# hjsuh94/irs_mpc

Hardware: AMD Instinct MI355X
Metric: rollouts*timesteps/s (randomized-smoothing pass) + iLQR-iters/s (higher is better)
Workload: dtype f32

## Files before the change

### irs_mpc_amd/csrc/ctrlbox_mfma.hip

```cpp
#include "boxqp.hpp"

namespace {

typedef double v4d __attribute__((ext_vector_type(4)));
typedef const __attribute__((address_space(1))) double* gptr_d;

constexpr int kPdasIterM = 10;
constexpr int kPdasSingleM = 50;
#ifndef IRS_LAZY_MIN
#define IRS_LAZY_MIN 6
#endif
constexpr int kLazyPrefixMin = IRS_LAZY_MIN;
constexpr int KIND_ABS_M = 0, KIND_REL_M = 1;

__device__ __forceinline__ double fast_rcp_m(double d) {
    double r = __builtin_amdgcn_rcp(d);
    r = fma(fma(-d, r, 1.0), r, r);
    r = fma(fma(-d, r, 1.0), r, r);
    return r;
}
__device__ __forceinline__ double readlane_d(double v, int src) {
    const int lo = __builtin_amdgcn_readlane(__double2loint(v), src);
    const int hi = __builtin_amdgcn_readlane(__double2hiint(v), src);
    return __hiloint2double(hi, lo);
}
template <int N>
__device__ __forceinline__ double row_newbcast_d(double v) {
    int lo = __double2loint(v), hi = __double2hiint(v);
    lo = __builtin_amdgcn_update_dpp(0, lo, 0x150 + N, 0xf, 0xf, true);
    hi = __builtin_amdgcn_update_dpp(0, hi, 0x150 + N, 0xf, 0xf, true);
    return __hiloint2double(hi, lo);
}
__device__ __forceinline__ double wmax_d(double v) {
#pragma unroll
    for (int s = 32; s >= 1; s >>= 1) v = fmax(v, __shfl_xor(v, s, 64));
    return v;
}
__device__ __forceinline__ double wmin_d(double v) {
#pragma unroll
    for (int s = 32; s >= 1; s >>= 1) v = fmin(v, __shfl_xor(v, s, 64));
    return v;
}
__device__ __forceinline__ int wmax_i(int v) {
#pragma unroll
    for (int s = 32; s >= 1; s >>= 1) v = max(v, __shfl_xor(v, s, 64));
    return v;
}
__device__ __forceinline__ int wmin_i(int v) {
#pragma unroll
    for (int s = 32; s >= 1; s >>= 1) v = min(v, __shfl_xor(v, s, 64));
    return v;
}

template <int NR, int M>
struct MfLayout {
    static constexpr int NS = NR + M, NH = NS + 1, NHP = (NH + 3) / 4 * 4, KA = NHP / 4;
    static constexpr bool FITS = NHP + M <= 16 && M <= 4;
    static constexpr int GR = NHP + M, GT = KA * 4 * GR, PT = KA * 4 * NHP;
    static __host__ __device__ size_t oG(int) { return 0; }
    static __host__ __device__ size_t oP(int T) { return (size_t)T * GT; }
    static __host__ __device__ size_t oV(int T) { return oP(T) + (size_t)(T + 1) * PT; }
    static __host__ __device__ size_t oQ(int T) { return oV(T) + (size_t)7 * T * M; }
    static __host__ __device__ size_t oS(int T) { return oQ(T) + (size_t)(T + 1) * NR; }
    static __host__ __device__ size_t rec_doubles(int T) { return oS(T) + (size_t)T; }
    static constexpr int small = 2 * NR * NR + M * M + NH + M + 16 + 128;
};

template <class Model, int KIND, bool LDSREC>
__global__ __launch_bounds__(128) void ctrlbox_mfma_kernel(BoxArgs a, double* gws, long long* stamps) {
    constexpr int NR = Model::NX, M = Model::NU;
    using L = MfLayout<NR, M>;
    constexpr int NS = L::NS, NH = L::NH, NHP = L::NHP, KA = L::KA, RN = L::KA;
    static_assert(L::FITS, "one 16 x 16 tile");
    constexpr double INF = __builtin_huge_val();
    extern __shared__ double lds[];
    const int T = a.T, lane = threadIdx.x & 63, col = lane & 15, rg = lane >> 4;
    const int wave = __builtin_amdgcn_readfirstlane((int)(threadIdx.x >> 6));
    const double tol_ = a.eps;
#ifdef IRS_CBM_STAMPS
    long long st_acc[24] = {0, 0, 0, 0, 0, 0, 0, 0, 0, 0, 0, 0, 0, 0, 0, 0, 0, 0, 0, 0, 0, 0, 0, 0};
#define CBM_MARK(k) do { const long long st_now = __builtin_amdgcn_s_memtime(); st_acc[k] += st_now - st_mark; st_mark = st_now; } while (0)
#define CBM_T0() const long long st_t0 = __builtin_amdgcn_s_memtime()
#define CBM_ADD(k, n) do { st_acc[k] += __builtin_amdgcn_s_memtime() - st_t0; st_acc[(k) + 1] += (n); } while (0)
#else
#define CBM_T0() do {} while (0)
#define CBM_MARK(k) do {} while (0)
#define CBM_ADD(k, n) do {} while (0)
#endif

    double* rec = LDSREC ? lds : gws;
    double* sm = LDSREC ? lds + L::rec_doubles(T) : lds;
    double* Gt = rec + L::oG(T);
    double* Pt = rec + L::oP(T);
    double* Vv = rec + L::oV(T);
    double* act_ = Vv;
    double* lo_ = Vv + (size_t)T * M;
    double* hi_ = Vv + (size_t)2 * T * M;
    double* uu_ = Vv + (size_t)3 * T * M;
    double* us_ = Vv + (size_t)4 * T * M;
    double* mu_ = Vv + (size_t)5 * T * M;
    double* bnd_ = Vv + (size_t)6 * T * M;
    double* qsd = rec + L::oQ(T);
    double* sig_ = rec + L::oS(T);
    double* Qsym = sm;
    double* Qdsym = Qsym + NR * NR;
    double* Rsym = Qdsym + NR * NR;
    double* sstart = Rsym + M * M;
    double* uctl = sstart + NH;
    double* junk = uctl + M + 16;

    auto rsync = [&]() {
        if constexpr (LDSREC) {
            asm volatile("s_waitcnt lgkmcnt(0)" ::: "memory");
        } else {
            __builtin_amdgcn_fence(__ATOMIC_RELEASE, "workgroup");
            asm volatile("s_waitcnt vmcnt(0) lgkmcnt(0)" ::: "memory");
            __builtin_amdgcn_fence(__ATOMIC_ACQUIRE, "workgroup");
        }
        __builtin_amdgcn_wave_barrier();
    };

    auto wg_barrier = [&]() {
        asm volatile("s_waitcnt vmcnt(0) lgkmcnt(0)" ::: "memory");
        __builtin_amdgcn_s_barrier();
        asm volatile("" ::: "memory");
    };

    if (wave == 1) {
        double xr[NR], ur[M], xn[NR], up[M], ub[M];
        if (lane == 0 && a.cost) *reinterpret_cast<unsigned long long*>(a.cost) = 0x7ff8000000000000ull;
#pragma unroll
        for (int i = 0; i < NR; ++i) xr[i] = a.x0[i];
#pragma unroll
        for (int j = 0; j < M; ++j) up[j] = 0.0;
        if (lane == 0) {
#pragma unroll
            for (int i = 0; i < NR; ++i) a.x_new[i] = xr[i];
        }
        auto quad = [&](const double* Wq, const double* e, int Kd) -> double {
            double q = 0.0;
            for (int i = 0; i < Kd; ++i)
                for (int j = 0; j < Kd; ++j) q += e[i] * Wq[i * Kd + j] * e[j];
            return q;
        };
        auto publish_start = [&]() {
#pragma unroll
            for (int j = 0; j < M; ++j) {
                double v = xr[0];
#pragma unroll
                for (int i = 1; i < NR; ++i) v = (i == Model::u_into_x(j)) ? xr[i] : v;
                ub[j] = v;
            }
            if (lane < NH) {
                double v = xr[0];
#pragma unroll
                for (int i = 1; i < NR; ++i) v = (i == lane) ? xr[i] : v;
#pragma unroll
                for (int j = 0; j < M; ++j) v = (NR + j == lane) ? ub[j] : v;
                sstart[lane] = lane == NS ? 1.0 : v;
            }
        };
        double cost = 0.0;
        unsigned warm = ~0u;
        irs_step_prepared<Model> pre;
        wg_barrier();
        publish_start();
        double xs[NR], dv[M];
        auto book = [&](int tau) {
            double e[NR];
#pragma unroll
            for (int i = 0; i < NR; ++i) e[i] = xs[i] - a.xd[(size_t)tau * NR + i];
            cost += quad(Qsym, e, NR) + quad(Rsym, dv, M);
            if (lane == 0) {
#pragma unroll
                for (int j = 0; j < M; ++j) a.u_new[(size_t)tau * M + j] = up[j];
#pragma unroll
                for (int i = 0; i < NR; ++i) a.x_new[(size_t)(tau + 1) * NR + i] = xr[i];
            }
        };
        for (int tau = 0; tau < T; ++tau) {
            wg_barrier();
            if (tau > 0) book(tau - 1);
            irs_step_along_prepare<Model>(a.p, xr, warm, pre);
            wg_barrier();
#pragma unroll
            for (int j = 0; j < M; ++j) ur[j] = KIND == KIND_ABS_M ? uctl[j] : ub[j] + uctl[j];
#pragma unroll
            for (int j = 0; j < M; ++j) dv[j] = ur[j] - (tau == 0 ? ub[j] : up[j]);
#pragma unroll
            for (int i = 0; i < NR; ++i) xs[i] = xr[i];
            irs_step_along_finish<Model>(a.p, xr, ur, pre, xn, &warm);
#pragma unroll
            for (int i = 0; i < NR; ++i) xr[i] = xn[i];
#pragma unroll
            for (int j = 0; j < M; ++j) up[j] = ur[j];
            publish_start();
        }
        book(T - 1);
        {
            double e[NR];
#pragma unroll
            for (int i = 0; i < NR; ++i) e[i] = xr[i] - a.xd[(size_t)T * NR + i];
            cost += quad(Qdsym, e, NR);
        }
        if (lane == 0 && a.cost) a.cost[0] = cost;
        return;
    }

    if (lane == 0) {
        a.info[0] = -1; a.info[1] = -1; a.info[2] = -1;
    }
    for (int q = lane; q < NR * NR; q += 64) {
        const int i = q / NR, j = q % NR;
        Qsym[q] = 0.5 * (a.Q[i * NR + j] + a.Q[j * NR + i]);
        Qdsym[q] = 0.5 * (a.Qd[i * NR + j] + a.Qd[j * NR + i]);
    }
    for (int q = lane; q < M * M; q += 64) {
        const int i = q / M, j = q % M;
        Rsym[q] = 0.5 * (a.R[i * M + j] + a.R[j * M + i]);
    }
    asm volatile("s_waitcnt lgkmcnt(0)" ::: "memory");
    __builtin_amdgcn_wave_barrier();
    const double* blo = KIND == KIND_ABS_M ? a.ulo : a.dlo;
    const double* bhi = KIND == KIND_ABS_M ? a.uhi : a.dhi;
    const int bs = KIND == KIND_ABS_M ? a.su : a.sd;
    for (int q = lane; q < T * M; q += 64) {
        const double lo = blo ? blo[(size_t)(q / M) * bs + q % M] : -INF;
        const double hi = bhi ? bhi[(size_t)(q / M) * bs + q % M] : INF;
        lo_[q] = lo;
        hi_[q] = hi;
        double a0 = a.act_io ? a.act_io[q] : 0.0;
        a0 = a0 < 0.0 ? (lo > -INF ? -1.0 : 0.0) : (a0 > 0.0 ? (hi < INF ? 1.0 : 0.0) : 0.0);
        act_[q] = a0;
        bnd_[q] = a0 < 0.0 ? lo : hi;
        uu_[q] = 0.0; us_[q] = 0.0; mu_[q] = 0.0;
    }
    for (int q = lane; q < (T + 1) * NR; q += 64) {
        const int t = q / NR, i = q % NR;
        double s = 0.0;
        for (int j = 0; j < NR; ++j) s += Qsym[i * NR + j] * a.xd[(size_t)t * NR + j];
        qsd[q] = -s;
    }
    for (size_t q = lane; q < (size_t)T * L::GT; q += 64) Gt[q] = 0.0;
    for (int q = lane; q < T; q += 64) sig_[q] = -1.0;
    auto Ru = [&](int i, int j) { return Rsym[i * M + j]; };
    v4d Lc;
#pragma unroll
    for (int r = 0; r < 4; ++r) {
        const int row = rg + 4 * r;
        double v = 0.0;
        if (row < NR && col < NR) v = Qsym[row * NR + col];
        else if (row >= NHP && row < NHP + M && col >= NHP && col < NHP + M) v = Ru(row - NHP, col - NHP);
        if (KIND == KIND_ABS_M) {
            if (row >= NR && row < NS && col >= NR && col < NS) v = Ru(row - NR, col - NR);
            else if (row >= NR && row < NS && col >= NHP && col < NHP + M) v = -Ru(row - NR, col - NHP);
            else if (col >= NR && col < NS && row >= NHP && row < NHP + M) v = -Ru(row - NHP, col - NR);
        }
        Lc[r] = v;
    }
    if (col < NHP) {
#pragma unroll
        for (int r = 0; r < KA; ++r) {
            const int row = rg + 4 * r;
            double v = 0.0;
            if (row < NR && col < NR) v = Qdsym[row * NR + col];
            else if ((col == NS && row < NR) || (row == NS && col < NR)) {
                const int i = col == NS ? row : col;
                for (int j = 0; j < NR; ++j) v -= Qdsym[i * NR + j] * a.xd[(size_t)T * NR + j];
            }
            Pt[(size_t)T * L::PT + (r * 4 + rg) * NHP + col] = v;
        }
    }
    rsync();

    gptr_d fp[5];
    int fstr[5];
    double fc[5];
    bool fld[5];
    {
        const gptr_d gA = (gptr_d)a.At, gB = (gptr_d)a.Bt, gc_ = (gptr_d)a.ct;
#pragma unroll
        for (int r = 0; r < 5; ++r) { fp[r] = gc_; fstr[r] = 0; fc[r] = 0.0; fld[r] = false; }
#pragma unroll
        for (int r = 0; r < 4; ++r) {
            const int row = rg + 4 * r;
            if (row < NR) {
                if (col < NR) { fp[r] = gA + row * NR + col; fstr[r] = NR * NR; fld[r] = true; }
                else if (col < NS) {
                    if (KIND == KIND_REL_M) { fp[r] = gB + row * M + (col - NR); fstr[r] = NR * M; fld[r] = true; }
                } else if (col == NS) { fp[r] = gc_ + row; fstr[r] = NR; fld[r] = true; }
                else if (col >= NHP && col < NHP + M) { fp[r] = gB + row * M + (col - NHP); fstr[r] = NR * M; fld[r] = true; }
            } else if (row < NS) {
                if (KIND == KIND_REL_M && col == row) fc[r] = 1.0;
                else if (col == NHP + (row - NR)) fc[r] = 1.0;
            } else if (row == NS && col == NS) {
                fc[r] = 1.0;
            }
        }
        if (rg < M) {
            if (col < NR) { fp[4] = gB + col * M + rg; fstr[4] = NR * M; fld[4] = true; }
            else if (col < NS) fc[4] = (col - NR) == rg ? 1.0 : 0.0;
        }
    }
    auto load_F = [&](int t, double* v) {
#pragma unroll
        for (int r = 0; r < 5; ++r) v[r] = fp[r][(long)t * fstr[r]];
    };
    auto finish_F = [&](const double* v, v4d& F, double& Ba) {
#pragma unroll
        for (int r = 0; r < 4; ++r) F[r] = fld[r] ? v[r] : fc[r];
        Ba = fld[4] ? v[4] : fc[4];
    };
    int qidx[KA];
    bool qhas[KA];
#pragma unroll
    for (int r = 0; r < KA; ++r) {
        const int row = rg + 4 * r;
        qhas[r] = (col == NS && row < NR) || (row == NS && col < NR);
        qidx[r] = qhas[r] ? (col == NS ? row : col) : 0;
    }

    int bad = 0;
    auto backward_sweep = [&](int t_hi, int t_lo) {
        if (t_hi < t_lo) return;
        CBM_T0();
        v4d P = {0.0, 0.0, 0.0, 0.0};
        if (col < NHP) {
#pragma unroll
            for (int r = 0; r < KA; ++r) P[r] = Pt[(size_t)(t_hi + 1) * L::PT + (r * 4 + rg) * NHP + col];
        }
        struct Pre { double Fraw[5]; double ac[M], bd[M], q[KA]; };
        auto load_step = [&](int t, Pre& p) {
            load_F(t, p.Fraw);
#pragma unroll
            for (int j = 0; j < M; ++j) {
                p.ac[j] = act_[(size_t)t * M + j];
                p.bd[j] = bnd_[(size_t)t * M + j];
            }
#pragma unroll
            for (int r = 0; r < KA; ++r) p.q[r] = qsd[(size_t)t * NR + qidx[r]];
        };
        bool pend = false;
        int pend_t = 0;
        v4d pendAcl = {0.0, 0.0, 0.0, 0.0};
        double pendGk = 0.0;
        auto flush_P = [&]() {
            double* pp = col < NHP ? Pt + (size_t)pend_t * L::PT + (size_t)rg * NHP + col : junk + lane;
            const int ps = col < NHP ? 4 * NHP : 0;
#pragma unroll
            for (int r = 0; r < KA; ++r) pp[r * ps] = P[r];
        };
        auto flush_G = [&]() {
            double* G = Gt + (size_t)pend_t * L::GT;
            double* gq = col < NH ? G + (size_t)col * L::GR + rg : junk + 64 + lane;
            const int gs = col < NH ? 4 : 0;
#pragma unroll
            for (int r = 0; r < KA; ++r) gq[r * gs] = pendAcl[r];
            double* gk = (col < NH && rg < M) ? G + (size_t)col * L::GR + NHP + rg : junk + 64 + lane;
            *gk = pendGk;
        };
        auto bw_step = [&](int t, const Pre& cur, Pre& nxt, bool prefetch) {
#ifdef IRS_CBM_STAMPS
            {
                const long long w0 = __builtin_amdgcn_s_memtime();
                asm volatile("s_waitcnt vmcnt(0)" ::: "memory");
                st_acc[7] += __builtin_amdgcn_s_memtime() - w0;
            }
#endif
#ifdef IRS_CBM_STAMPS
            long long st_mark = __builtin_amdgcn_s_memtime();
#endif
            v4d F;
            double Ba;
            finish_F(cur.Fraw, F, Ba);
            double ac[M], bb[M];
#pragma unroll
            for (int j = 0; j < M; ++j) {
                ac[j] = cur.ac[j];
                bb[j] = cur.bd[j];
            }
            v4d Lt = Lc;
            v4d D1 = {0.0, 0.0, 0.0, 0.0};
            v4d Th;
            if constexpr (LDSREC && KA == 3) {
                D1 = __builtin_amdgcn_mfma_f64_16x16x4f64(P[0], F[0], D1, 0, 0, 0);
                if (pend) flush_P();
                __builtin_amdgcn_sched_barrier(0);
                D1 = __builtin_amdgcn_mfma_f64_16x16x4f64(P[1], F[1], D1, 0, 0, 0);
                if (pend) flush_G();
                __builtin_amdgcn_sched_barrier(0);
                D1 = __builtin_amdgcn_mfma_f64_16x16x4f64(P[2], F[2], D1, 0, 0, 0);
                if (prefetch) load_F(t - 1, nxt.Fraw);
#pragma unroll
                for (int r = 0; r < KA; ++r) Lt[r] = qhas[r] ? cur.q[r] : Lc[r];
                __builtin_amdgcn_sched_barrier(0);
                Th = __builtin_amdgcn_mfma_f64_16x16x4f64(F[0], D1[0], Lt, 0, 0, 0);
                if (prefetch) {
#pragma unroll
                    for (int j = 0; j < M; ++j) {
                        nxt.ac[j] = act_[(size_t)(t - 1) * M + j];
                        nxt.bd[j] = bnd_[(size_t)(t - 1) * M + j];
                    }
                }
                __builtin_amdgcn_sched_barrier(0);
                Th = __builtin_amdgcn_mfma_f64_16x16x4f64(F[1], D1[1], Th, 0, 0, 0);
                if (prefetch) {
#pragma unroll
                    for (int r = 0; r < KA; ++r) nxt.q[r] = qsd[(size_t)(t - 1) * NR + qidx[r]];
                }
                __builtin_amdgcn_sched_barrier(0);
                Th = __builtin_amdgcn_mfma_f64_16x16x4f64(F[2], D1[2], Th, 0, 0, 0);
            } else if constexpr (LDSREC && KA == 2) {
                D1 = __builtin_amdgcn_mfma_f64_16x16x4f64(P[0], F[0], D1, 0, 0, 0);
                if (pend) flush_P();
                __builtin_amdgcn_sched_barrier(0);
                D1 = __builtin_amdgcn_mfma_f64_16x16x4f64(P[1], F[1], D1, 0, 0, 0);
                if (pend) flush_G();
                if (prefetch) load_F(t - 1, nxt.Fraw);
#pragma unroll
                for (int r = 0; r < KA; ++r) Lt[r] = qhas[r] ? cur.q[r] : Lc[r];
                __builtin_amdgcn_sched_barrier(0);
                Th = __builtin_amdgcn_mfma_f64_16x16x4f64(F[0], D1[0], Lt, 0, 0, 0);
                if (prefetch) {
#pragma unroll
                    for (int j = 0; j < M; ++j) {
                        nxt.ac[j] = act_[(size_t)(t - 1) * M + j];
                        nxt.bd[j] = bnd_[(size_t)(t - 1) * M + j];
                    }
#pragma unroll
                    for (int r = 0; r < KA; ++r) nxt.q[r] = qsd[(size_t)(t - 1) * NR + qidx[r]];
                }
                __builtin_amdgcn_sched_barrier(0);
                Th = __builtin_amdgcn_mfma_f64_16x16x4f64(F[1], D1[1], Th, 0, 0, 0);
            } else {
#pragma unroll
                for (int r = 0; r < KA; ++r) Lt[r] = qhas[r] ? cur.q[r] : Lc[r];
                if (prefetch) load_step(t - 1, nxt);
                if constexpr (LDSREC) {
                    D1 = __builtin_amdgcn_mfma_f64_16x16x4f64(P[0], F[0], D1, 0, 0, 0);
                    if (pend) flush_P();
                    __builtin_amdgcn_sched_barrier(0);
                    if constexpr (KA >= 2) D1 = __builtin_amdgcn_mfma_f64_16x16x4f64(P[1], F[1], D1, 0, 0, 0);
                    if (pend) flush_G();
                    __builtin_amdgcn_sched_barrier(0);
#pragma unroll
                    for (int s = 2; s < KA; ++s) D1 = __builtin_amdgcn_mfma_f64_16x16x4f64(P[s], F[s], D1, 0, 0, 0);
                } else {
#pragma unroll
                    for (int s = 0; s < KA; ++s) D1 = __builtin_amdgcn_mfma_f64_16x16x4f64(P[s], F[s], D1, 0, 0, 0);
                }
                Th = Lt;
#pragma unroll
                for (int s = 0; s < KA; ++s) Th = __builtin_amdgcn_mfma_f64_16x16x4f64(F[s], D1[s], Th, 0, 0, 0);
            }
            asm volatile("" :: "v"(Th[0]), "v"(Th[RN]));
            CBM_MARK(8);
            bool allpin = true;
#pragma unroll
            for (int j = 0; j < M; ++j) allpin = allpin && ac[j] != 0.0;
            double Kb = 0.0;
            bool my_free = false;
            if (__builtin_amdgcn_readfirstlane((int)allpin)) {
#pragma unroll
                for (int i = 0; i < M; ++i)
                    if (i == rg) Kb = col == NS ? bb[i] : 0.0;
                if constexpr (LDSREC) {
                    double* sp = lane == 0 ? sig_ + t : junk + lane;
                    *sp = 1.0;
                } else if (lane == 0) {
                    sig_[t] = 1.0;
                }
                CBM_MARK(9);
            } else {
                double H[M][M], gc[M], mf[M], bz[M];
                const v4d zero4 = {0.0, 0.0, 0.0, 0.0};
                const v4d Gc = __builtin_amdgcn_mfma_f64_16x16x4f64(rg == (col >> 2) ? 1.0 : 0.0, Th[RN], zero4, 0, 0, 0);
                auto bc = [&](double v, int j) {
                    switch (j) {
                        case 0: return row_newbcast_d<NHP + 0>(v);
                        case 1: return row_newbcast_d<(NHP + 1) & 15>(v);
                        case 2: return row_newbcast_d<(NHP + 2) & 15>(v);
                        default: return row_newbcast_d<(NHP + 3) & 15>(v);
                    }
                };
#pragma unroll
                for (int i = 0; i < M; ++i) {
#pragma unroll
                    for (int j = i; j < M; ++j) {
                        H[i][j] = bc(Gc[i], j);
                        H[j][i] = H[i][j];
                    }
                    gc[i] = Gc[i];
                    mf[i] = ac[i] == 0.0 ? 1.0 : 0.0;
                    bz[i] = ac[i] == 0.0 ? 0.0 : bb[i];
                }
                asm volatile("" :: "v"(H[0][0]), "v"(gc[0]), "v"(gc[M - 1]));
                CBM_MARK(9);
                double Hm[M][M], Hi[M][M], y[M];
    #pragma unroll
                for (int i = 0; i < M; ++i)
    #pragma unroll
                    for (int j = 0; j < M; ++j) Hm[i][j] = H[i][j];
                bool anypin = false;
    #pragma unroll
                for (int j = 0; j < M; ++j) anypin = anypin || ac[j] != 0.0;
                const bool pins = __builtin_amdgcn_readfirstlane((int)anypin) != 0;
                if (pins) {
    #pragma unroll
                    for (int i = 0; i < M; ++i)
    #pragma unroll
                        for (int j = 0; j < M; ++j) Hm[i][j] = i == j ? (ac[i] == 0.0 ? H[i][i] : 1.0) : H[i][j] * (mf[i] * mf[j]);
                }
                const double hsel = col == NS ? 1.0 : 0.0;
                double rhs[M];
    #pragma unroll
                for (int i = 0; i < M; ++i) {
                    rhs[i] = gc[i];
                }
                if (pins) {
    #pragma unroll
                    for (int i = 0; i < M; ++i) {
                        double hb0 = 0.0, hb1 = 0.0;
    #pragma unroll
                        for (int l = 0; l < M; ++l) {
                            if (l & 1) hb1 = fma(H[i][l], bz[l], hb1);
                            else hb0 = fma(H[i][l], bz[l], hb0);
                        }
                        rhs[i] = fma(hsel, hb0 + hb1, gc[i]) * mf[i];
                    }
                }
                bool spd = true;
                auto inv2 = [&](double p, double q, double r, double& ip, double& iq, double& ir) {
                    const double det = fma(p, r, -q * q);
                    spd = spd && p > 0.0 && det > 0.0;
                    const double id = fast_rcp_m(det);
                    ip = r * id; iq = -q * id; ir = p * id;
                };
                if constexpr (M == 1) {
                    spd = Hm[0][0] > 0.0;
                    Hi[0][0] = fast_rcp_m(Hm[0][0]);
                } else if constexpr (M == 2) {
                    inv2(Hm[0][0], Hm[0][1], Hm[1][1], Hi[0][0], Hi[0][1], Hi[1][1]);
                    Hi[1][0] = Hi[0][1];
                } else {
                    static_assert(M == 1 || M == 2 || M == 4, "closed-form inverse for 1, 2 or 4 controls");
                    double a0, a1, a2;
                    inv2(Hm[0][0], Hm[0][1], Hm[1][1], a0, a1, a2);
                    const double w00 = fma(a0, Hm[0][2], a1 * Hm[1][2]), w01 = fma(a0, Hm[0][3], a1 * Hm[1][3]);
                    const double w10 = fma(a1, Hm[0][2], a2 * Hm[1][2]), w11 = fma(a1, Hm[0][3], a2 * Hm[1][3]);
                    const double s00 = Hm[2][2] - fma(Hm[0][2], w00, Hm[1][2] * w10);
                    const double s01 = Hm[2][3] - fma(Hm[0][2], w01, Hm[1][2] * w11);
                    const double s11 = Hm[3][3] - fma(Hm[0][3], w01, Hm[1][3] * w11);
                    double c0, c1, c2;
                    inv2(s00, s01, s11, c0, c1, c2);
                    const double t0 = fma(a0, rhs[0], a1 * rhs[1]), t1 = fma(a1, rhs[0], a2 * rhs[1]);
                    const double q0 = rhs[2] - fma(Hm[0][2], t0, Hm[1][2] * t1);
                    const double q1 = rhs[3] - fma(Hm[0][3], t0, Hm[1][3] * t1);
                    y[2] = fma(c0, q0, c1 * q1);
                    y[3] = fma(c1, q0, c2 * q1);
                    y[0] = t0 - fma(w00, y[2], w01 * y[3]);
                    y[1] = t1 - fma(w10, y[2], w11 * y[3]);
                }
                if (!spd && bad == 0) bad = t + 1;
                if constexpr (M != 4) {
    #pragma unroll
                    for (int i = 0; i < M; ++i) {
                        double y0 = 0.0, y1 = 0.0;
    #pragma unroll
                        for (int l = 0; l < M; ++l) {
                            if (l & 1) y1 = fma(Hi[i][l], rhs[l], y1);
                            else y0 = fma(Hi[i][l], rhs[l], y0);
                        }
                        y[i] = y0 + y1;
                    }
                }
                double mfree = 0.0;
    #pragma unroll
                for (int i = 0; i < M; ++i) {
                    const double kv = hsel * bz[i] - y[i];
                    if (i == rg) { Kb = kv; mfree = mf[i]; }
                }
                if (rg >= M || col >= NH) Kb = 0.0;
                my_free = mfree != 0.0;
            }
            asm volatile("" :: "v"(Kb));
            CBM_MARK(10);
            v4d D = __builtin_amdgcn_mfma_f64_16x16x4f64(Th[RN], Kb, Th, 0, 0, 0);
            v4d Pn = __builtin_amdgcn_mfma_f64_16x16x4f64(Kb, D[RN], D, 0, 0, 0);
            v4d Acl = __builtin_amdgcn_mfma_f64_16x16x4f64(Ba, Kb, F, 0, 0, 0);
#pragma unroll
            for (int r = 0; r < 4; ++r) {
                const int row = rg + 4 * r;
                if constexpr (NH == NHP) P[r] = r < KA ? Pn[r] : 0.0;
                else P[r] = (r < KA && row < NH && col < NH) ? Pn[r] : 0.0;
            }
            double* G = Gt + (size_t)t * L::GT;
            if constexpr (LDSREC) {
                pend = true;
                pend_t = t;
                pendAcl = Acl;
                pendGk = my_free ? Kb : D[RN];
            } else {
                if (col < NHP) {
#pragma unroll
                    for (int r = 0; r < KA; ++r) Pt[(size_t)t * L::PT + (r * 4 + rg) * NHP + col] = P[r];
                }
                if (col < NH) {
#pragma unroll
                    for (int r = 0; r < KA; ++r) G[col * L::GR + (rg + 4 * r)] = Acl[r];
                    if (rg < M) G[col * L::GR + (NHP + rg)] = my_free ? Kb : D[RN];
                }
            }
            asm volatile("" :: "v"(P[0]));
            CBM_MARK(11);
        
        };
        Pre pa, pb;
        load_step(t_hi, pa);
        int t = t_hi;
        for (; t - 1 >= t_lo; t -= 2) {
            bw_step(t, pa, pb, true);
            bw_step(t - 1, pb, pa, t - 2 >= t_lo);
        }
        if (t >= t_lo) bw_step(t, pa, pb, false);
        if constexpr (LDSREC) {
            if (pend) {
                flush_P();
                flush_G();
            }
        }
        rsync();
        CBM_ADD(0, t_hi - t_lo + 1);
    };

    auto policy_rollout = [&](int t0, double* dst, int te, bool clip = false) {
        CBM_T0();
        v4d S = {0.0, 0.0, 0.0, 0.0};
        if (col == 0) {
#pragma unroll
            for (int s = 0; s < KA; ++s) {
                const int k = rg + 4 * s;
                S[s] = k < NH ? sstart[k] : 0.0;
            }
        }
        const int gofs = col < L::GR ? col : 0;
        const bool out_lane = col == 0 && rg < M;
        const int cj = rg < M ? rg : 0;
        struct Fw { double g[KA]; double ti, lo, hi, ac; };
        auto roll_range = [&](int ta, int tb, v4d& S, bool clipping) {
            const double* gp = Gt + (size_t)ta * L::GT + (size_t)rg * L::GR + gofs;
            int tq = ta;
            auto fetch = [&](Fw& f) {
#pragma unroll
                for (int s = 0; s < KA; ++s) f.g[s] = gp[4 * s * L::GR];
                gp += L::GT;
                if (clipping) {
                    f.ti = (double)tq;
                    f.lo = lo_[(size_t)tq * M + cj];
                    f.hi = hi_[(size_t)tq * M + cj];
                    f.ac = act_[(size_t)tq * M + cj];
                    ++tq;
                }
            };
            double* mo = (out_lane || !LDSREC) ? mu_ + (size_t)ta * M + (rg < M ? rg : 0) : junk + lane;
            const int mstride = (out_lane || !LDSREC) ? M : 0;
            auto emit = [&](const v4d& Dp) {
                if constexpr (LDSREC) *mo = Dp[RN];
                else if (out_lane) *mo = Dp[RN];
                mo += mstride;
            };
            auto step = [&](const Fw& f, const v4d& Sin, v4d& Sout, bool has_prev) {
                v4d Dn = {0.0, 0.0, 0.0, 0.0};
                Dn = __builtin_amdgcn_mfma_f64_16x16x4f64(col < L::GR ? f.g[0] : 0.0, Sin[0], Dn, 0, 0, 0);
                if (has_prev) emit(Sin);
#pragma unroll
                for (int s = 1; s < KA; ++s)
                    Dn = __builtin_amdgcn_mfma_f64_16x16x4f64(col < L::GR ? f.g[s] : 0.0, Sin[s], Dn, 0, 0, 0);
                if (clipping) {
                    const double raw = Dn[RN];
                    const double cl = fmin(fmax(raw, f.lo), f.hi);
                    const double dlt = (out_lane && f.ac == 0.0) ? cl - raw : 0.0;
                    if (__ballot(dlt != 0.0) != 0ull) {
                        const double bav = fp[4][(long)(int)f.ti * fstr[4]];
                        Dn = __builtin_amdgcn_mfma_f64_16x16x4f64(fld[4] ? bav : fc[4], dlt, Dn, 0, 0, 0);
                    }
                }
                Sout = Dn;
            };
            Fw fa, fb;
            v4d S1;
            fetch(fa);
            int t = ta;
            bool hp = false;
            for (; t + 1 < tb; t += 2) {
                fetch(fb);
                step(fa, S, S1, hp);
                if (t + 2 < tb) fetch(fa);
                step(fb, S1, S, true);
                hp = true;
            }
            if (t < tb) {
                step(fa, S, S1, hp);
                emit(S1);
                S = S1;
            } else if (hp) {
                emit(S);
            }
        };
#ifdef IRS_CBM_STAMPS
        const long long st_fl0 = __builtin_amdgcn_s_memtime();
#endif
        if (!clip) {
            roll_range(t0, te, S, false);
        } else {
            #ifndef IRS_KCHECK
#define IRS_KCHECK 16
#endif
            constexpr int kCheck = IRS_KCHECK;
            int t = t0;
            bool found = false;
            while (t < te && !found) {
                const int tc = min(t + kCheck, te);
                const v4d Ssave = S;
                roll_range(t, tc, S, false);
#ifdef IRS_CBM_STAMPS
                st_acc[20] += tc - t;
                st_acc[21] += 1;
#endif
                rsync();
                bool v = false;
                for (int q = t * M + lane; q < tc * M; q += 64) {
                    const double raw = mu_[q];
                    v = v || (act_[q] == 0.0 && (raw < lo_[q] || raw > hi_[q]));
                }
                if (__any(v)) {
                    S = Ssave;
                    found = true;
                } else {
                    t = tc;
                }
            }
#ifdef IRS_CBM_STAMPS
            st_acc[19] += te - t;
#endif
            if (t < te) roll_range(t, te, S, true);
        }
#ifdef IRS_CBM_STAMPS
        asm volatile("" :: "v"(S[0]));
        st_acc[13] += __builtin_amdgcn_s_memtime() - st_fl0;
        st_acc[12] += 1;
#endif
        rsync();
        for (int q = t0 * M + lane; q < te * M; q += 64) {
            const double raw = mu_[q], ac = act_[q];
            const double bd = bnd_[q];
            dst[q] = ac == 0.0 ? raw : bd;
            mu_[q] = ac == 0.0 ? 0.0 : raw;
        }
        rsync();
        CBM_ADD(2, te - t0);
    };

    auto saturated_start = [&](int t0) {
        v4d S = {0.0, 0.0, 0.0, 0.0};
        if (col == 0) {
#pragma unroll
            for (int s = 0; s < KA; ++s) {
                const int k = rg + 4 * s;
                S[s] = k < NH ? sstart[k] : 0.0;
            }
        }
        const gptr_d gB = (gptr_d)a.Bt;
        for (int t = t0; t < T; ++t) {
            const double* G = Gt + (size_t)t * L::GT;
            v4d Dn = {0.0, 0.0, 0.0, 0.0};
#pragma unroll
            for (int s = 0; s < KA; ++s) {
                const double g = col < L::GR ? G[(4 * s + rg) * L::GR + (col < L::GR ? col : 0)] : 0.0;
                Dn = __builtin_amdgcn_mfma_f64_16x16x4f64(g, S[s], Dn, 0, 0, 0);
            }
            double dlt[M];
#pragma unroll
            for (int j = 0; j < M; ++j) {
                const double v = readlane_d(Dn[RN], 16 * j);
                const double lo = lo_[(size_t)t * M + j], hi = hi_[(size_t)t * M + j];
                const double c = fmin(fmax(v, lo), hi);
                dlt[j] = c - v;
                if (lane == 0) {
                    act_[(size_t)t * M + j] = v < lo - tol_ ? -1.0 : (v > hi + tol_ ? 1.0 : 0.0);
                    bnd_[(size_t)t * M + j] = v < lo - tol_ ? lo : hi;
                    sig_[t] = -1.0;
                }
            }
            if (col == 0) {
#pragma unroll
                for (int s = 0; s < KA; ++s) {
                    const int row = rg + 4 * s;
                    double corr = 0.0;
                    if (row < NR) {
#pragma unroll
                        for (int j = 0; j < M; ++j) corr += gB[((size_t)t * NR + row) * M + j] * dlt[j];
                    } else if (row < NS) {
#pragma unroll
                        for (int j = 0; j < M; ++j) corr = (row - NR == j) ? dlt[j] : corr;
                    }
                    S[s] = Dn[s] + corr;
                }
            }
        }
        rsync();
    };

#ifdef IRS_CBM_STAMPS
    const long long st_begin = __builtin_amdgcn_s_memtime();
#endif
    int it_max = 0, n_fail = 0;
    const double tol = a.eps;
    bool full = true;
    wg_barrier();

    for (int tau = 0; tau < T; ++tau) {
        {
            CBM_T0();
            wg_barrier();
            CBM_ADD(4, 1);
        }
        const int t0 = tau;
        if (tau == 0) {
            bool any = false;
            for (int q = lane; q < T * M; q += 64) any = any || act_[q] != 0.0;
            if (!__any(any)) {
                backward_sweep(T - 1, 0);
                saturated_start(0);
            }
        }
        int t_dirty = full ? T - 1 : t0 - 1;
        int iters = 0;
        bool conv = false;
        int stale_hi = t0 - 1;
        auto prefix_end = [&]() {
            int pe = t0 - 1;
            for (int base = t0; base < T; base += 64) {
                const int t = base + lane;
                bool ok = false;
                if (t < T) {
                    bool allp = sig_[t] == 1.0;
#pragma unroll
                    for (int j = 0; j < M; ++j) allp = allp && act_[(size_t)t * M + j] != 0.0;
                    ok = allp;
                }
                const unsigned long long bal = __ballot(ok);
                const int run = bal == ~0ull ? 64 : __builtin_ctzll(~bal);
                pe = base + run - 1;
                if (run < 64) break;
            }
            return pe;
        };
        for (int it = 0; it < kPdasIterM + kPdasSingleM && !conv; ++it) {
            ++iters;
            const bool single = it >= kPdasIterM;
            int pe = t0 - 1;
            if (KIND == KIND_ABS_M && max(t_dirty, stale_hi) >= t0) {
                pe = prefix_end();
                if (pe - t0 + 1 < kLazyPrefixMin) pe = t0 - 1;
            }
            {
                const int hi = max(t_dirty, stale_hi), lo = max(t0, pe + 1);
                if (hi >= lo) backward_sweep(hi, lo);
                if (hi >= t0) stale_hi = lo - 1;
            }
            policy_rollout(t0, uu_, T, KIND == KIND_ABS_M);
            int chg = -1;
            double rworst = 0.0;
            int rq = 0x7fffffff;
            for (int qb = t0 * M; qb < T * M; qb += 64) {
                const int q = qb + lane;
                bool changed = false;
                if (q < T * M) {
                    const double ac = act_[q], u = uu_[q], mu = mu_[q];
                    const bool fresh = q / M > stale_hi;
                    double nw = ac;
                    if (ac == 0.0) {
                        if (u < lo_[q] - tol) nw = -1.0;
                        else if (u > hi_[q] + tol) nw = 1.0;
                    } else if (ac < 0.0) {
                        if (fresh && mu < -tol) nw = 0.0;
                    } else {
                        if (fresh && mu > tol) nw = 0.0;
                    }
                    if (single && nw == 0.0 && ac != 0.0) {
                        const double v = fabs(mu);
                        if (v > rworst) { rworst = v; rq = q; }
                        nw = ac;
                    }
                    changed = nw != ac;
                    if (changed) { act_[q] = nw; bnd_[q] = nw < 0.0 ? lo_[q] : hi_[q]; sig_[q / M] = -1.0; }
                }
                const unsigned long long cb = __ballot(changed);
                if (cb != 0ull) chg = max(chg, (qb + 63 - __builtin_clzll(cb)) / M);
            }
            if (single) {
                const double wm = wmax_d(rworst);
                if (wm > 0.0) {
                    const int qw = wmin_i(rworst == wm ? rq : 0x7fffffff);
                    if (lane == 0) { act_[qw] = 0.0; sig_[qw / M] = -1.0; }
                    chg = max(chg, qw / M);
                }
            }
            rsync();
            if (chg < 0 && stale_hi >= t0) {
                const int ph = stale_hi;
#ifdef IRS_CBM_STAMPS
                st_acc[14] += ph - t0 + 1;
#endif
                backward_sweep(ph, t0);
                stale_hi = t0 - 1;
                policy_rollout(t0, uu_, ph + 1);
                for (int qb = t0 * M; qb < (ph + 1) * M; qb += 64) {
                    const int q = qb + lane;
                    bool rel = false;
                    if (q < (ph + 1) * M) {
                        const double ac = act_[q], mu = mu_[q];
                        rel = (ac < 0.0 && mu < -tol) || (ac > 0.0 && mu > tol);
                        if (rel) { act_[q] = 0.0; sig_[q / M] = -1.0; }
                    }
                    const unsigned long long cb = __ballot(rel);
                    if (cb != 0ull) chg = max(chg, (qb + 63 - __builtin_clzll(cb)) / M);
                }
                rsync();
#ifdef IRS_CBM_STAMPS
                st_acc[15] += chg >= 0 ? 1 : 0;
#endif
            }
            if (chg < 0) conv = true;
            else t_dirty = chg;
        }
        if (stale_hi >= t0) { t_dirty = max(t_dirty, stale_hi); stale_hi = t0 - 1; }
        if (!conv) {
#ifdef IRS_CBM_STAMPS
            st_acc[16] += 1;
            st_acc[18] += iters;
#endif
            int chg = -1;
            for (int q = t0 * M + lane; q < T * M; q += 64) {
                const double lo = lo_[q], hi = hi_[q];
                const double u = fmin(fmax(uu_[q], lo), hi);
                uu_[q] = u;
                const double nw = u <= lo ? -1.0 : (u >= hi ? 1.0 : 0.0);
                if (nw != act_[q]) { act_[q] = nw; bnd_[q] = nw < 0.0 ? lo : hi; sig_[q / M] = -1.0; chg = max(chg, q / M); }
            }
            chg = wmax_i(chg);
            rsync();
            t_dirty = max(t_dirty, chg);
            for (int it2 = 0; it2 < a.max_iter && !conv; ++it2) {
                ++iters;
                backward_sweep(t_dirty, t0);
                t_dirty = t0 - 1;
                policy_rollout(t0, us_, T);
                double best = INF;
                int bq = 0x7fffffff;
                for (int q = t0 * M + lane; q < T * M; q += 64) {
                    if (act_[q] == 0.0) {
                        const double u = uu_[q], d = us_[q] - u;
                        double room = INF;
                        if (d > 0.0) room = (hi_[q] - u) / d;
                        else if (d < 0.0) room = (lo_[q] - u) / d;
                        if (room < best) { best = room; bq = q; }
                    }
                }
                const double alpha = wmin_d(best);
                if (alpha < 1.0) {
                    const int qb = wmin_i(best == alpha ? bq : 0x7fffffff);
                    for (int q = t0 * M + lane; q < T * M; q += 64) {
                        const double u = uu_[q], d = us_[q] - u;
                        if (q == qb) {
                            act_[q] = d > 0.0 ? 1.0 : -1.0;
                            uu_[q] = d > 0.0 ? hi_[q] : lo_[q];
                            bnd_[q] = uu_[q];
                            sig_[q / M] = -1.0;
                        } else {
                            uu_[q] = u + alpha * d;
                        }
                    }
                    rsync();
                    t_dirty = qb / M;
                    continue;
                }
                double worst = 0.0;
                int wq = 0x7fffffff;
                for (int q = t0 * M + lane; q < T * M; q += 64) {
                    uu_[q] = us_[q];
                    const double ac = act_[q], mu = mu_[q];
                    const double viol = ac < 0.0 ? -mu : (ac > 0.0 ? mu : 0.0);
                    if (viol > worst) { worst = viol; wq = q; }
                }
                const double wmax = wmax_d(worst);
                if (wmax <= tol) {
                    rsync();
                    conv = true;
                } else {
                    const int qw = wmin_i(worst == wmax ? wq : 0x7fffffff);
                    if (lane == 0) { act_[qw] = 0.0; sig_[qw / M] = -1.0; }
                    rsync();
                    t_dirty = qw / M;
                }
            }
        }
#ifdef IRS_CBM_STAMPS
        st_acc[17] += iters;
#endif
        it_max = max(it_max, iters);
        n_fail += conv ? 0 : 1;
        full = !conv;
        if (tau == 0 && a.act_io != nullptr) {
            for (int q = lane; q < T * M; q += 64) a.act_io[q] = act_[q];
        }
        if (lane < M) {
            const size_t q = (size_t)tau * M + lane;
            uctl[lane] = fmin(fmax(uu_[q], lo_[q]), hi_[q]);
        }
        wg_barrier();
    }
    if (lane == 0) {
        a.info[0] = bad; a.info[1] = it_max; a.info[2] = n_fail;
    }
#ifdef IRS_CBM_STAMPS
    if (lane == 0 && stamps != nullptr) {
        st_acc[6] = __builtin_amdgcn_s_memtime() - st_begin;
        for (int k = 0; k < 24; ++k) stamps[k] = st_acc[k];
    }
#endif
}

#ifdef IRS_CBM_STAMPS
static long long* g_stamps = nullptr;
static long long* cbm_stamps() {
    if (g_stamps == nullptr) {
        (void)hipMalloc(reinterpret_cast<void**>(&g_stamps), 24 * sizeof(long long));
        (void)hipMemset(g_stamps, 0, 24 * sizeof(long long));
    }
    return g_stamps;
}
#else
static long long* cbm_stamps() { return nullptr; }
#endif

template <class Model, int KIND>
int launch_ctrlbox_mfma(const BoxArgs& a, const BoxPlan& p, double* ws, hipStream_t st) {
    if (p.place == BoxPlace::TilesLds) {
        constexpr auto kern = ctrlbox_mfma_kernel<Model, KIND, true>;
        const int rc = irs_raise_lds_limit<kern>(p.lds, "irs_quasistatic_box_descent");
        if (rc != IRS_OK) return rc;
        hipLaunchKernelGGL(kern, dim3(1), dim3(128), p.lds, st, a, (double*)nullptr, cbm_stamps());
    } else {
        auto kern = ctrlbox_mfma_kernel<Model, KIND, false>;
        hipLaunchKernelGGL(kern, dim3(1), dim3(128), p.lds, st, a, ws, cbm_stamps());
    }
    return IRS_OK;
}

}

size_t irs_ctrlbox_mfma_record_bytes(int model, int T) {
    size_t r = 0;
    IRS_DISPATCH_MODEL(model, {
        if constexpr (has_u_into_x<Model>::value) {
            using L = MfLayout<Model::NX, Model::NU>;
            if constexpr (L::FITS) r = L::rec_doubles(T) * sizeof(double);
        }
    });
    return r;
}

size_t irs_ctrlbox_mfma_lds_bytes(int model, int T) {
    size_t r = 0;
    IRS_DISPATCH_MODEL(model, {
        if constexpr (has_u_into_x<Model>::value) {
            using L = MfLayout<Model::NX, Model::NU>;
            if constexpr (L::FITS) r = (L::rec_doubles(T) + L::small) * sizeof(double);
        }
    });
    return r;
}

int irs_ctrlbox_mfma_launch(int model, const BoxArgs& a, int kind, const BoxPlan& p, double* ws, hipStream_t st) {
    int rc = IRS_ERR_UNSUPPORTED;
    IRS_DISPATCH_MODEL(model, {
        if constexpr (has_u_into_x<Model>::value) {
            if constexpr (MfLayout<Model::NX, Model::NU>::FITS)
                rc = kind == KIND_ABS_M ? launch_ctrlbox_mfma<Model, KIND_ABS_M>(a, p, ws, st)
                                        : launch_ctrlbox_mfma<Model, KIND_REL_M>(a, p, ws, st);
        }
    });
    return rc;
}

#ifdef IRS_CBM_STAMPS
extern "C" void irs_cbm_print_stamps(void) {
    long long h[24];
    (void)hipDeviceSynchronize();
    if (g_stamps == nullptr || hipMemcpy(h, g_stamps, sizeof(h), hipMemcpyDeviceToHost) != hipSuccess) return;
    fprintf(stderr, "[cbm stamps] backward %lld cyc / %lld steps; forward %lld cyc / %lld steps; wait for plant %lld cyc / "
                    "%lld tails; MPC loop %lld cyc; of backward: waiting for the prefetched step data %lld cyc\n", h[0], h[1], h[2], h[3], h[4], h[5], h[6], h[7]);
    fprintf(stderr, "[cbm stamps] backward step phases: head+6 MFMA %lld, gather %lld, inverse+gains %lld, 3 MFMA+stores %lld cyc\n",
            h[8], h[9], h[10], h[11]);
    fprintf(stderr, "[cbm stamps] forward: %lld rollouts, %lld cyc inside their step loops; backward steps that re-swept a lazily skipped "
                    "pinned head: %lld (%lld of those sweeps released a component)\n", h[12], h[13], h[14], h[15]);
    fprintf(stderr, "[cbm stamps] active-set iterations over all tails: %lld; tails that left the primal-dual phase unconverged: %lld "
                    "(after %lld iterations)\n", h[17], h[16], h[18]);
    fprintf(stderr, "[cbm stamps] clipped rollouts: %lld plain steps in %lld chunks, %lld clipping steps\n", h[20], h[21], h[19]);
}
#endif
```

Before: 12.91 billion.

## Solve 4-control box-QP gains via MFMA-built cofactors instead of Schur inverse

For four controls, the backward-sweep gain solve changes. The old path gathered the full 4x4 Hessian per lane and inverted it with a Schur-complement 2x2 block inverse. The new path folds the pinned components into a masked bordered operand and builds cofactor rows with one MFMA plus quad-permute DPP moves. The gains then come from a second MFMA scaled by a reciprocal of the determinant, with a positivity/finiteness check replacing the SPD test. It also precomputes the active-set mask once via readfirstlane and adds stamp counters. The aim is to remove the per-lane Hessian gather and the scalar inverse work, at the cost of tricky lane-layout logic and possible numerical differences.

```diff
diff --git a/irs_mpc_amd/csrc/ctrlbox_mfma.hip b/irs_mpc_amd/csrc/ctrlbox_mfma.hip
--- a/irs_mpc_amd/csrc/ctrlbox_mfma.hip
+++ b/irs_mpc_amd/csrc/ctrlbox_mfma.hip
@@ -30,6 +30,16 @@
     lo = __builtin_amdgcn_update_dpp(0, lo, 0x150 + N, 0xf, 0xf, true);
     hi = __builtin_amdgcn_update_dpp(0, hi, 0x150 + N, 0xf, 0xf, true);
     return __hiloint2double(hi, lo);
+}
+template <int CTRL>
+__device__ __forceinline__ double quad_perm_d(double v) {
+    int lo = __double2loint(v), hi = __double2hiint(v);
+    lo = __builtin_amdgcn_update_dpp(0, lo, CTRL, 0xf, 0xf, true);
+    hi = __builtin_amdgcn_update_dpp(0, hi, CTRL, 0xf, 0xf, true);
+    return __hiloint2double(hi, lo);
+}
+__device__ __forceinline__ int pos_finite(double v) {
+    return (unsigned long long)__double_as_longlong(v) - 1ull < 0x7fefffffffffffffull ? 1 : 0;
 }
 __device__ __forceinline__ double wmax_d(double v) {
 #pragma unroll
@@ -319,6 +329,9 @@
         qhas[r] = (col == NS && row < NR) || (row == NS && col < NR);
         qidx[r] = qhas[r] ? (col == NS ? row : col) : 0;
     }
+    const int rsig = col >= 12 ? (col & 3) : (((col & 3) + 1 + (col >> 2)) & 3);
+    const double rsel4 = rg == rsig ? ((col >> 2) == 2 && (col & 1) ? -1.0 : 1.0) : 0.0;
+    const double dg4 = (col >= NHP && rg == (col & 3)) ? ((col & 1) ? -1.0 : 1.0) : 0.0;
 
     int bad = 0;
     auto backward_sweep = [&](int t_hi, int t_lo) {
@@ -329,7 +342,7 @@
 #pragma unroll
             for (int r = 0; r < KA; ++r) P[r] = Pt[(size_t)(t_hi + 1) * L::PT + (r * 4 + rg) * NHP + col];
         }
-        struct Pre { double Fraw[5]; double ac[M], bd[M], q[KA]; };
+        struct Pre { double Fraw[5]; double ac[M], bd[M], q[KA], br; };
         auto load_step = [&](int t, Pre& p) {
             load_F(t, p.Fraw);
 #pragma unroll
@@ -337,6 +350,7 @@
                 p.ac[j] = act_[(size_t)t * M + j];
                 p.bd[j] = bnd_[(size_t)t * M + j];
             }
+            if constexpr (M == 4) p.br = bnd_[(size_t)t * M + rg];
 #pragma unroll
             for (int r = 0; r < KA; ++r) p.q[r] = qsd[(size_t)t * NR + qidx[r]];
         };
@@ -401,6 +415,7 @@
                         nxt.ac[j] = act_[(size_t)(t - 1) * M + j];
                         nxt.bd[j] = bnd_[(size_t)(t - 1) * M + j];
                     }
+                    if constexpr (M == 4) nxt.br = bnd_[(size_t)(t - 1) * M + rg];
                 }
                 __builtin_amdgcn_sched_barrier(0);
                 Th = __builtin_amdgcn_mfma_f64_16x16x4f64(F[1], D1[1], Th, 0, 0, 0);
@@ -427,6 +442,7 @@
                         nxt.ac[j] = act_[(size_t)(t - 1) * M + j];
                         nxt.bd[j] = bnd_[(size_t)(t - 1) * M + j];
                     }
+                    if constexpr (M == 4) nxt.br = bnd_[(size_t)(t - 1) * M + rg];
 #pragma unroll
                     for (int r = 0; r < KA; ++r) nxt.q[r] = qsd[(size_t)(t - 1) * NR + qidx[r]];
                 }
@@ -453,6 +469,15 @@
 #pragma unroll
                 for (int s = 0; s < KA; ++s) Th = __builtin_amdgcn_mfma_f64_16x16x4f64(F[s], D1[s], Th, 0, 0, 0);
             }
+            int pm = 0;
+            double pinv = 0.0;
+            if constexpr (M == 4) {
+#pragma unroll
+                for (int j = 0; j < M; ++j) pm |= (ac[j] != 0.0 ? 1 : 0) << j;
+                pm = __builtin_amdgcn_readfirstlane(pm);
+                pinv = col == NS ? -cur.br : dg4;
+                asm volatile("" :: "v"(pinv));
+            }
             asm volatile("" :: "v"(Th[0]), "v"(Th[RN]));
             CBM_MARK(8);
             bool allpin = true;
@@ -460,7 +485,7 @@
             for (int j = 0; j < M; ++j) allpin = allpin && ac[j] != 0.0;
             double Kb = 0.0;
             bool my_free = false;
-            if (__builtin_amdgcn_readfirstlane((int)allpin)) {
+            if (M == 4 ? pm == (1 << M) - 1 : __builtin_amdgcn_readfirstlane((int)allpin) != 0) {
 #pragma unroll
                 for (int i = 0; i < M; ++i)
                     if (i == rg) Kb = col == NS ? bb[i] : 0.0;
@@ -470,7 +495,38 @@
                 } else if (lane == 0) {
                     sig_[t] = 1.0;
                 }
+                CBM_MARK(23);
+            } else if constexpr (M == 4) {
+                const bool pin_r = (pm >> rg) & 1;
+                const int keep = pin_r ? 0 : -1;
+                const int xhi = pin_r ? __double2hiint(pinv) : ((col >= NHP && (col & 1)) ? (int)0x80000000 : 0);
+                const int xlo = pin_r ? __double2loint(pinv) : 0;
+                const double bop = __hiloint2double((__double2hiint(Th[RN]) & keep) ^ xhi, (__double2loint(Th[RN]) & keep) ^ xlo);
+                const v4d zero4 = {0.0, 0.0, 0.0, 0.0};
+                const v4d Gr = __builtin_amdgcn_mfma_f64_16x16x4f64(rsel4, bop, zero4, 0, 0, 0);
+                double V[3][3];
+#pragma unroll
+                for (int a = 0; a < 3; ++a) {
+                    V[a][0] = quad_perm_d<0x39>(Gr[a]);
+                    V[a][1] = quad_perm_d<0x4e>(Gr[a]);
+                    V[a][2] = quad_perm_d<0x93>(Gr[a]);
+                }
+                asm volatile("" :: "v"(V[0][0]), "v"(V[2][2]));
+#ifdef IRS_CBM_STAMPS
+                st_acc[22] += 1;
+#endif
                 CBM_MARK(9);
+                const double m12 = fma(V[0][1], V[1][2], -V[0][2] * V[1][1]);
+                const double m02 = fma(V[0][0], V[1][2], -V[0][2] * V[1][0]);
+                const double m01 = fma(V[0][0], V[1][1], -V[0][1] * V[1][0]);
+                const double cf = fma(V[2][0], m12, fma(-V[2][1], m02, V[2][2] * m01));
+                const v4d Y = __builtin_amdgcn_mfma_f64_16x16x4f64(cf, bop, zero4, 0, 0, 0);
+                const double ndet = readlane_d(Y[RN], 63);
+                const int ok = pos_finite(V[0][0]) & pos_finite(-m01) & pos_finite(cf);
+                if (!(__builtin_amdgcn_readlane(ok, 63) & pos_finite(-ndet)) && bad == 0) bad = t + 1;
+                const double kpin = (pin_r && col == NS) ? cur.br : 0.0;
+                Kb = (pin_r || col >= NH) ? kpin : Y[RN] * fast_rcp_m(ndet);
+                my_free = !pin_r;
             } else {
                 double H[M][M], gc[M], mf[M], bz[M];
                 const v4d zero4 = {0.0, 0.0, 0.0, 0.0};
@@ -495,6 +551,9 @@
                     bz[i] = ac[i] == 0.0 ? 0.0 : bb[i];
                 }
                 asm volatile("" :: "v"(H[0][0]), "v"(gc[0]), "v"(gc[M - 1]));
+#ifdef IRS_CBM_STAMPS
+                st_acc[22] += 1;
+#endif
                 CBM_MARK(9);
                 double Hm[M][M], Hi[M][M], y[M];
     #pragma unroll
@@ -529,6 +588,7 @@
                         rhs[i] = fma(hsel, hb0 + hb1, gc[i]) * mf[i];
                     }
                 }
+                static_assert(M == 1 || M == 2, "closed-form inverse for 1 or 2 controls here, cofactors for 4 above");
                 bool spd = true;
                 auto inv2 = [&](double p, double q, double r, double& ip, double& iq, double& ir) {
                     const double det = fma(p, r, -q * q);
@@ -539,40 +599,20 @@
                 if constexpr (M == 1) {
                     spd = Hm[0][0] > 0.0;
                     Hi[0][0] = fast_rcp_m(Hm[0][0]);
-                } else if constexpr (M == 2) {
+                } else {
                     inv2(Hm[0][0], Hm[0][1], Hm[1][1], Hi[0][0], Hi[0][1], Hi[1][1]);
                     Hi[1][0] = Hi[0][1];
-                } else {
-                    static_assert(M == 1 || M == 2 || M == 4, "closed-form inverse for 1, 2 or 4 controls");
-                    double a0, a1, a2;
-                    inv2(Hm[0][0], Hm[0][1], Hm[1][1], a0, a1, a2);
-                    const double w00 = fma(a0, Hm[0][2], a1 * Hm[1][2]), w01 = fma(a0, Hm[0][3], a1 * Hm[1][3]);
-                    const double w10 = fma(a1, Hm[0][2], a2 * Hm[1][2]), w11 = fma(a1, Hm[0][3], a2 * Hm[1][3]);
-                    const double s00 = Hm[2][2] - fma(Hm[0][2], w00, Hm[1][2] * w10);
-                    const double s01 = Hm[2][3] - fma(Hm[0][2], w01, Hm[1][2] * w11);
-                    const double s11 = Hm[3][3] - fma(Hm[0][3], w01, Hm[1][3] * w11);
-                    double c0, c1, c2;
-                    inv2(s00, s01, s11, c0, c1, c2);
-                    const double t0 = fma(a0, rhs[0], a1 * rhs[1]), t1 = fma(a1, rhs[0], a2 * rhs[1]);
-                    const double q0 = rhs[2] - fma(Hm[0][2], t0, Hm[1][2] * t1);
-                    const double q1 = rhs[3] - fma(Hm[0][3], t0, Hm[1][3] * t1);
-                    y[2] = fma(c0, q0, c1 * q1);
-                    y[3] = fma(c1, q0, c2 * q1);
-                    y[0] = t0 - fma(w00, y[2], w01 * y[3]);
-                    y[1] = t1 - fma(w10, y[2], w11 * y[3]);
                 }
                 if (!spd && bad == 0) bad = t + 1;
-                if constexpr (M != 4) {
     #pragma unroll
-                    for (int i = 0; i < M; ++i) {
-                        double y0 = 0.0, y1 = 0.0;
+                for (int i = 0; i < M; ++i) {
+                    double y0 = 0.0, y1 = 0.0;
     #pragma unroll
-                        for (int l = 0; l < M; ++l) {
-                            if (l & 1) y1 = fma(Hi[i][l], rhs[l], y1);
-                            else y0 = fma(Hi[i][l], rhs[l], y0);
-                        }
-                        y[i] = y0 + y1;
-                    }
+                    for (int l = 0; l < M; ++l) {
+                        if (l & 1) y1 = fma(Hi[i][l], rhs[l], y1);
+                        else y0 = fma(Hi[i][l], rhs[l], y0);
+                    }
+                    y[i] = y0 + y1;
                 }
                 double mfree = 0.0;
     #pragma unroll
@@ -1109,5 +1149,7 @@
     fprintf(stderr, "[cbm stamps] active-set iterations over all tails: %lld; tails that left the primal-dual phase unconverged: %lld "
                     "(after %lld iterations)\n", h[17], h[16], h[18]);
     fprintf(stderr, "[cbm stamps] clipped rollouts: %lld plain steps in %lld chunks, %lld clipping steps\n", h[20], h[21], h[19]);
-}
-#endif
+    fprintf(stderr, "[cbm stamps] backward steps with a free component: %lld (phases gather, inverse+gains); fully pinned: %lld cyc "
+                    "between head and 3 MFMA\n", h[22], h[23]);
+}
+#endif
```

Result: no change. 12.85 billion, median of 4 (-0.5%).
